# jean-pierreBoth/hnswlib-rs

Measured on AMD Instinct MI355X. Metric: queries/sec (+ recall@10), batched HNSW search, higher is better.
Workload: dtype f32

## Files before the change

### hnswlib-rs_amd/csrc/search_device.hip

```cpp
#include <hip/hip_runtime.h>

#include <algorithm>
#include <chrono>
#include <cmath>
#include <cstdio>
#include <cstdlib>
#include <cstring>
#include <thread>
#include <vector>

#include "hnswio.hpp"
#include "search_device.hpp"
#include "search_kernels.hpp"
#include "worker_pool.hpp"

namespace hnswgpu {

namespace {
Knobs read_knobs() {
    Knobs k;
    auto num = [](const char* name, int unset) { const char* e = std::getenv(name); return e ? std::atoi(e) : unset; };
    auto flag = [](const char* name) { return std::getenv(name) != nullptr; };
    k.hash_bits = num("HNSWGPU_HASH_BITS", -1);
    k.no_sched = flag("HNSWGPU_NO_SCHED");
// ... 614 lines not shown
        HIP_TRY(hipEventElapsedTime(&ms, w.ev_start, w.ev_stop));
        HIP_TRY(hipEventElapsedTime(&ms_main, w.ev_ks, w.ev_stop));
        info.ms = ms;
        info.main_ms = ms_main;
        info.launches = 1;
        publish();
        drain.done = true;
        return OK;
    }

    HIP_TRY(w.tie.ensure(nq * sizeof(uint32_t)));
    HIP_TRY(w.retry[0].ensure(nq * sizeof(uint32_t)));
    HIP_TRY(w.retry[1].ensure(nq * sizeof(uint32_t)));

    int slots = 1;
    while ((uint64_t)slots * 64 < ef) slots *= 2;
    if (slots == 8) slots = 16;
    if (v_.deg_stride > 64u) slots = 16;

    const uint32_t idbits = std::max<uint32_t>(1u, ceil_log2(v_.n));
    const uint64_t expect = ef * std::min<uint64_t>(v_.deg_stride, 64);
    uint32_t tbits = std::min<uint32_t>(14u, std::max<uint32_t>(8u, ceil_log2(expect)));
    {
        std::lock_guard<std::mutex> g(meta_mu_);
        if (adapt_ef_ == ef && adapt_tbits_ != 0) tbits = adapt_tbits_;
    }
    bool env_forced = false;
    const Knobs& kn = knobs();
    if (kn.hash_bits >= 6 && kn.hash_bits <= 14) { tbits = (uint32_t)kn.hash_bits; env_forced = true; }
    const uint32_t tbits_first = tbits;
    const size_t lds_fixed = tile_bytes + IDS_BYTES;
    int table = TABLE_LDS_CELL16;
    bool grown = false;

    const bool scheduled = nq >= 256 && !kn.no_sched;
    if (scheduled) {
        HIP_TRY(w.order.ensure(nq * sizeof(uint32_t)));
        HIP_TRY(kernel_set(kernel_metric()).launch_order(stream, w.pre.as<PreDescent>(), (uint32_t)nq, w.order.as<uint32_t>()));
    }
    uint32_t launches = 0, stop_recorded_after = ~0u;
    uint32_t work = (uint32_t)nq;
    uint32_t n_flagged = 0, n_literal = 0;
    const uint32_t* qlist = scheduled ? w.order.as<uint32_t>() : nullptr;
    int pingpong = 0;
    bool all_done = false;
    const bool pair_auto = (kernel_metric() == DIST_COSINE || kernel_metric() == DIST_DOT) && v_.row_stride <= 32u && strict_ties &&
                           nq >= PAIR_SEARCH_AUTO_MIN_QUERIES;
    if (kn.pair_search > 0 || (kn.pair_search < 0 && pair_auto)) {
        const int tbp = (int)tbits + kn.pair_tbits_delta;
        const uint32_t tb = (uint32_t)std::max(6, std::min<int>(tbp, (int)std::min(14u, idbits + 3u)));
        const bool ok = ef <= 128 && v_.deg_stride <= 64u && kernel_metric() < KM_SIMD8_FIRST && nq >= 512 && idbits >= tb - 3u && idbits - (tb - 3u) <= 13u &&
                        idbits - (tb - 3u) >= 1u;
        if (ok) {
            const KernelSet& ks = kernel_set(kernel_metric());
            SearchArgs a{};
            a.tbits = tb;
            a.restbits = idbits - (tb - 3u);
            a.idbits = idbits;
            a.tile_bytes = tile_bytes;
            a.nrm2 = static_cast<const double*>(d_nrm2_);
            const size_t lds = pair_lds_bytes(tile_bytes, tb, (uint32_t)ef);
            int per_cu = 0;
            HIP_TRY(ks.pair_occupancy(lds, &per_cu));
            if (per_cu >= 1) {
                if (kn.pair_wg_per_cu > 0) per_cu = std::min(per_cu, kn.pair_wg_per_cu);
                const uint64_t npairs = (nq + 1) / 2;
                const uint32_t grid = (uint32_t)std::min<uint64_t>((uint64_t)per_cu * (uint64_t)num_cu_, npairs);
                if (kn.trace_launch)
                    std::fprintf(stderr, "[hnswgpu launch] pair pass: %u queries, %d workgroups per CU, %zu bytes of LDS each, tables 2^%u cells\n",
                                 work, per_cu, lds, tb);
                a.queries = w.qpad.as<float>();
                a.qlist = qlist;
                a.nq = work;
                a.k = (uint32_t)k;
                a.ef = (uint32_t)ef;
                a.work_counter = static_cast<uint32_t*>(w.d_ctrl);
                a.overflow_count = static_cast<uint32_t*>(w.d_ctrl) + 1;
                a.retry_out = w.retry[pingpong].as<uint32_t>();
                a.out_ids = d_out_ids;
                a.out_dists = d_out_dists;
                a.out_layer = d_out_layer;
                a.out_rank = d_out_rank;
                a.out_counts = d_out_counts;
                a.id_stride = layout.id_stride;
                a.dist_stride = layout.dist_stride;
                a.count_stride = layout.count_stride;
                a.stats = stats;
                a.pre = w.pre.as<PreDescent>();
                a.tie_list = w.tie.as<uint32_t>();
                a.pair_ties_to_retry = strict_ties ? 1u : 0u;
                {
                    a.bitmap_words = (v_.n + 31) / 32;
                    const uint64_t slice = (uint64_t)a.bitmap_words * sizeof(uint32_t);
                    const uint64_t blocks = std::min<uint64_t>(2ull * grid, std::max<uint64_t>(2, (4ull << 30) / slice));
                    HIP_TRY(w.bitmap.ensure(blocks * slice));
                    a.bitmap = w.bitmap.as<uint32_t>();
                    a.bitmap_blocks = (uint32_t)blocks;
                }
                HIP_TRY(ks.launch_pair(grid, lds, stream, v_, a, LaunchEvents{w.ev_ks, w.ev_ke}));
                ++launches;
                volatile uint32_t* ctrl = static_cast<volatile uint32_t*>(w.h_ctrl);
                HIP_TRY(hipMemcpyAsync(w.h_ctrl, w.d_ctrl, 24, hipMemcpyDeviceToHost, stream));
                HIP_TRY(hipEventRecord(w.ev_stop, stream));
                stop_recorded_after = launches;
                HIP_TRY(wait_stream(stream));
                n_flagged = ctrl[4];
                info.pair_retries = ctrl[1];
                if (table != TABLE_GLOBAL_BITMAP && !env_forced) {
                    uint32_t next = tbits_first;
                    if ((uint64_t)ctrl[2] * 8 > nq && tbits_first < 14u) next = tbits_first + 1;
                    else if ((uint64_t)ctrl[3] * 32 < nq && tbits_first > 8u) next = tbits_first - 1;
                    std::lock_guard<std::mutex> g(meta_mu_);
                    adapt_ef_ = ef;
                    adapt_tbits_ = next;
                }
                if (ctrl[1] == 0) {
                    all_done = true;
                } else {
                    work = ctrl[1];
                    qlist = w.retry[pingpong].as<uint32_t>();
                    pingpong ^= 1;
                }
            }
        }
    }
    while (!all_done) {
        SearchArgs a{};
        size_t lds = lds_fixed;
        if (table != TABLE_GLOBAL_BITMAP) {
            uint32_t tb = std::max(3u, std::min(tbits, idbits + 3u));
            if (idbits - (tb - 3u) <= 13u) {
                table = TABLE_LDS_CELL16;
                a.restbits = idbits - (tb - 3u);
                lds += (size_t)2 << tb;
            } else {
                table = TABLE_LDS_CELL32;
                lds += (size_t)4 << tb;
            }
            a.tbits = tb;
        }
        a.tile_bytes = tile_bytes;
        a.nrm2 = static_cast<const double*>(d_nrm2_);
        a.idbits = idbits;
        const KernelSet& ks = kernel_set(kernel_metric());
        const bool strict_kernel = strict_ties && table != TABLE_GLOBAL_BITMAP && !kn.no_inkernel;
        if (slots <= (strict_kernel ? HNSW_MERGE_SMAX : HNSW_MERGE_LEAN_SMAX)) {
            a.merge_entries = (uint32_t)slots * 64u + 64u;
            lds += (size_t)a.merge_entries * sizeof(hent_t);
        }
        int per_cu = 0;
        int strict_cap = STRICT_WG_PER_CU;
        if (kn.strict_wg_per_cu > 0) strict_cap = kn.strict_wg_per_cu;
        if (strict_kernel) {
            a.cand_lds = 256;
            if (kn.cand_lds >= 0) {
                a.cand_lds = (uint32_t)std::min(4096, kn.cand_lds);
            } else {
                int occ256 = 0, occ512 = 0;
                HIP_TRY(ks.occupancy(slots, table, true, lds + 256 * sizeof(hent_t), &occ256));
                HIP_TRY(ks.occupancy(slots, table, true, lds + 512 * sizeof(hent_t), &occ512));
                if (std::min(occ512, strict_cap) >= std::min(occ256, strict_cap)) a.cand_lds = 512;
            }
            lds += (size_t)a.cand_lds * sizeof(hent_t);
        }
        HIP_TRY(ks.occupancy(slots, table, strict_kernel, lds, &per_cu));
        if (per_cu < 1) per_cu = 1;
        if (strict_kernel) per_cu = std::min(per_cu, strict_cap);
        if (kn.waves_per_cu > 0) per_cu = std::max(1, std::min(per_cu, kn.waves_per_cu));
        uint32_t grid = (uint32_t)std::min<uint64_t>((uint64_t)per_cu * (uint64_t)num_cu_, work);
        if (kn.trace_launch)
            std::fprintf(stderr, "[hnswgpu launch] %u queries, %d workgroups per CU (strict cap %d), %zu bytes of LDS each (literal heap: %u entries), table 2^%u cells, strict %d, work list %s, slots %d, visited set %s\n",
                         work, per_cu, strict_cap, lds, a.cand_lds, a.tbits, (int)strict_kernel,
                         qlist ? "sorted" : "input order", slots,
                         table == TABLE_LDS_CELL16 ? "cell16" : table == TABLE_LDS_CELL32 ? "cell32" : "bitmap");
        a.queries = w.qpad.as<float>();
        a.qlist = qlist;
        a.nq = work;
        a.k = (uint32_t)k;
        a.ef = (uint32_t)ef;
        a.work_counter = static_cast<uint32_t*>(w.d_ctrl);
        a.overflow_count = static_cast<uint32_t*>(w.d_ctrl) + 1;
        a.retry_out = w.retry[pingpong].as<uint32_t>();
        a.out_ids = d_out_ids;
        a.out_dists = d_out_dists;
        a.out_layer = d_out_layer;
        a.out_rank = d_out_rank;
        a.out_counts = d_out_counts;
        a.id_stride = layout.id_stride;
        a.dist_stride = layout.dist_stride;
        a.count_stride = layout.count_stride;
        a.stats = stats;
        a.pre = w.pre.as<PreDescent>();
        {
            a.bitmap_words = (v_.n + 31) / 32;
            const uint64_t slice = (uint64_t)a.bitmap_words * sizeof(uint32_t);
            uint64_t blocks = std::min<uint64_t>(grid, std::max<uint64_t>(1, (4ull << 30) / slice));
            if (table == TABLE_GLOBAL_BITMAP) grid = (uint32_t)blocks;
            HIP_TRY(w.bitmap.ensure(blocks * slice));
            a.bitmap = w.bitmap.as<uint32_t>();
            a.bitmap_blocks = (uint32_t)blocks;
        }
        a.tie_list = w.tie.as<uint32_t>();
        if (strict_kernel) {
            const uint32_t cap = 4096;
            const uint64_t need = (uint64_t)grid * cap * sizeof(hent_t);
            HIP_TRY(w.cand.ensure(need));
            HIP_TRY(w.oplog.ensure(need));
            a.cand_scratch = w.cand.as<hent_t>();
            a.cand_cap = cap;
            a.oplog = w.oplog.as<hent_t>();
            a.oplog_cap = cap;
            if (kn.exact_first >= 0) a.exact_first = kn.exact_first != 0 ? 1u : 0u;
        }
        if (launches != 0) HIP_TRY(hipMemsetAsync(w.d_ctrl, 0, 16, stream));
        HIP_TRY(ks.launch_search(slots, table, strict_kernel, grid, lds, stream, v_, a,
                                 launches == 0 ? LaunchEvents{w.ev_ks, w.ev_ke} : LaunchEvents{}));
        ++launches;
        volatile uint32_t* ctrl = static_cast<volatile uint32_t*>(w.h_ctrl);
        HIP_TRY(hipMemcpyAsync(w.h_ctrl, w.d_ctrl, 24, hipMemcpyDeviceToHost, stream));
        HIP_TRY(hipEventRecord(w.ev_stop, stream));
        stop_recorded_after = launches;
        HIP_TRY(wait_stream(stream));
        n_flagged = ctrl[4];
        n_literal += ctrl[5];
        if (launches == 1 && table != TABLE_GLOBAL_BITMAP && !env_forced && nq >= 256) {
            uint32_t next = tbits_first;
            if ((uint64_t)ctrl[2] * 8 > nq && tbits_first < 14u) next = tbits_first + 1;
            else if ((uint64_t)ctrl[3] * 32 < nq && tbits_first > 8u) next = tbits_first - 1;
            std::lock_guard<std::mutex> g(meta_mu_);
            adapt_ef_ = ef;
            adapt_tbits_ = next;
        }
        if (ctrl[1] == 0) break;
        work = ctrl[1];
        qlist = w.retry[pingpong].as<uint32_t>();
        pingpong ^= 1;
        if (table == TABLE_GLOBAL_BITMAP) { err = "internal error: bitmap visited set reported an overflow"; return ERR_DEVICE; }
        if (!grown && tbits < 14u) {
            tbits = std::min<uint32_t>(14u, tbits + 2u);
            grown = true;
        } else {
            table = TABLE_GLOBAL_BITMAP;
        }
    }
    info.ties = n_flagged + n_literal;
    if (strict_ties && n_flagged > 0) {
        int rc = run_exact(w, w.qpad.as<float>(), w.tie.as<uint32_t>(), n_flagged, k, ef, nullptr, d_out_ids, d_out_dists, d_out_layer,
                           d_out_rank, d_out_counts, stats, stream, nullptr, err, layout);
        if (rc != OK) return rc;
        ++launches;
    }
    if (stop_recorded_after != launches) {
        HIP_TRY(hipEventRecord(w.ev_stop, stream));
        HIP_TRY(wait_event(w.ev_stop));
    }
    float ms = 0.f, ms_main = 0.f;
    HIP_TRY(hipEventElapsedTime(&ms, w.ev_start, w.ev_stop));
    HIP_TRY(hipEventElapsedTime(&ms_main, w.ev_ks, w.ev_ke));
    info.ms = ms;
    info.main_ms = ms_main;
    info.launches = launches;
    publish();
    drain.done = true;
    return OK;
}

namespace {
struct HostCall {
    const float* queries;
    const float* const* rows;
    float* hq;
    uint64_t d, nq, chunk_rows, task_rows, tasks_per_chunk, n_chunks;
    std::atomic<uint64_t> next_gather{0};
    std::vector<std::atomic<uint32_t>> chunk_left;
    std::atomic<int> phase{0};
    std::atomic<uint64_t> next_unpack{0};
    uint64_t unpack_rows = 256;
    DeviceIndex::HostAnswers answers{};
    const uint32_t* stats = nullptr;
    uint8_t* flags = nullptr;
    const DeviceIndex::AnswerSink* sink = nullptr;
    double us_gather = 0., us_unpack = 0.;

    HostCall(uint64_t n_chunks_) : chunk_left(n_chunks_) {}
    bool gather_one() {
        const uint64_t t = next_gather.fetch_add(1, std::memory_order_relaxed);
        if (t >= n_chunks * tasks_per_chunk) return false;
        const uint64_t c = t / tasks_per_chunk, lo = c * chunk_rows + (t % tasks_per_chunk) * task_rows;
        const uint64_t hi = std::min({nq, (c + 1) * chunk_rows, lo + task_rows});
        const uint64_t row_bytes = d * sizeof(float);
        if (lo < hi) {
            if (queries) std::memcpy(hq + lo * d, queries + lo * d, (hi - lo) * row_bytes);
            else for (uint64_t i = lo; i < hi; ++i) std::memcpy(hq + i * d, rows[i], row_bytes);
        }
        chunk_left[c].fetch_sub(1, std::memory_order_release);
        return true;
    }
    void unpack_all() {
        for (;;) {
            const uint64_t lo = next_unpack.fetch_add(unpack_rows, std::memory_order_relaxed);
            if (lo >= nq) break;
            const uint64_t hi = std::min(nq, lo + unpack_rows);
            if (flags) for (uint64_t i = lo; i < hi; ++i) flags[i] = stats[i * 8 + 3] == 6u ? 1 : 0;
            sink->rows(sink->ctx, answers, lo, hi);
        }
    }
    static std::atomic<int>& calls_in_flight() {
        static std::atomic<int> n{0};
        return n;
    }
    struct InFlight {
        InFlight() { calls_in_flight().fetch_add(1, std::memory_order_relaxed); }
        ~InFlight() { calls_in_flight().fetch_sub(1, std::memory_order_relaxed); }
    };
    struct Spin {
        std::chrono::steady_clock::time_point t0 = std::chrono::steady_clock::now();
        unsigned n = 0;
        bool napping = false;
    };
    static void relax(Spin& w) {
        if (!w.napping) {
#if defined(__x86_64__) || defined(__i386__)
            __builtin_ia32_pause();
#else
            std::this_thread::yield();
// ... 451 lines not shown
```

### hnswlib-rs_amd/csrc/search_kernels.hpp

```cpp
#pragma once
#include <hip/hip_runtime.h>
#include <hip/hip_ext.h>
#include <cstdint>
#include "search_device.hpp"

namespace hnswgpu {

constexpr uint32_t EXPANDED = 0x80000000u;
constexpr uint32_t EMPTY_SLOT = 0xFFFFFFFFu;
constexpr int TABLE_LDS_CELL16 = 0;
constexpr int TABLE_LDS_CELL32 = 1;
constexpr int TABLE_GLOBAL_BITMAP = 2;

constexpr int KM_SIMD8_FIRST = 7;
constexpr int KM_L2_SIMD8 = 7, KM_COSINE_SIMD8 = 8, KM_DOT_SIMD8 = 9, KM_L1_SIMD8 = 10;
constexpr int KM_COUNT = 11;
inline int simd8_kernel_metric(int dist) {
    return dist == DIST_L2 ? KM_L2_SIMD8 : dist == DIST_COSINE ? KM_COSINE_SIMD8 : dist == DIST_DOT ? KM_DOT_SIMD8 : dist == DIST_L1 ? KM_L1_SIMD8 : -1;
}

constexpr uint32_t IDS_BYTES = 64 * 4;

typedef unsigned long long hent_t;

struct PreDescent {
    uint32_t pivot;
    uint32_t dcur_bits;
    uint32_t n_dist;
    uint32_t n_expand;
};
struct DescendArgs {
    const float* src;
    float* qpad;
    PreDescent* pre;
    uint32_t nq;
    uint32_t tile_bytes;
    const double* nrm2;
    uint32_t* ctrl;
    uint32_t ctrl_words;
    uint32_t pair;
};

struct SearchArgs {
    const float* queries;
    const uint32_t* qlist;
    uint32_t nq;
    uint32_t k;
    uint32_t ef;
    uint32_t tbits;
    uint32_t tile_bytes;
    uint32_t idbits;
    uint32_t restbits;
    uint32_t* work_counter;
    uint32_t* overflow_count;
    uint32_t* retry_out;
    uint32_t* bitmap;
    uint32_t bitmap_words;
    uint32_t bitmap_blocks;
    uint32_t* tie_list;
    hent_t* cand_scratch;
    uint32_t cand_cap;
    uint32_t cand_lds;
    uint32_t merge_entries;
    uint32_t exact_first;
    uint32_t pair_ties_to_retry;
    hent_t* oplog;
    uint32_t oplog_cap;
    const double* nrm2;
    uint64_t* out_ids;
    float* out_dists;
    uint8_t* out_layer;
    int32_t* out_rank;
    uint32_t* out_counts;
    const PreDescent* pre;
    uint32_t* stats;
    uint32_t id_stride, dist_stride, count_stride;
};

struct ExactArgs {
    hent_t* heaps;
    uint64_t heap_stride;
    uint32_t cand_cap;
    uint32_t r_lds_cap;
    uint32_t cand_lds;
    const uint32_t* allow;
};

struct BuildLists {
    uint32_t* lists[NB_LAYER_MAX];
    uint32_t stride[NB_LAYER_MAX];
};
struct BuildArgs {
    const float* vec;
    uint32_t row_stride;
    const uint32_t* lists[NB_LAYER_MAX];
    uint32_t stride[NB_LAYER_MAX];
    const uint8_t* level;
    const uint32_t* slot0;
    uint32_t first, count;
    uint32_t entry, entry_level;
    uint32_t layer_mask;
    uint32_t ef_c;
    uint32_t tbits, idbits, restbits, tile_bytes;
    uint32_t* bitmap;
    uint32_t bitmap_words, bitmap_blocks;
    uint32_t* work_counter;
    uint32_t* fail_count;
    uint32_t* out_ids;
    float* out_d;
    uint32_t* out_n;
    uint32_t* hit_ids;
    float* hit_d;
    const double* nrm2;
};

struct SelectArgs {
    const float* vec;
    uint32_t row_stride;
    uint32_t tile_bytes;
    const double* nrm2;
    uint32_t* cand_ids;
    const float* cand_d;
    const uint32_t* cand_n;
    uint32_t ef_c;
    const uint16_t* slot_nb;
    uint32_t n_slots;
    uint32_t sel_stride;
    uint32_t keep_pruned;
    uint32_t* sel_ids;
    float* sel_d;
    uint32_t* sel_n;
    uint32_t* work_counter;
};

constexpr uint32_t LAB_PUSH = 1, LAB_POP = 2, LAB_PUSH_LANES = 3, LAB_INSERT = 4, LAB_MERGE = 5, LAB_BATCH = 6, LAB_VISIT = 7;
struct LaneLabArgs {
    const uint32_t* ops;
    uint32_t n_ops;
    const uint32_t* lanes;
    uint32_t mode;
    uint32_t p0, p1, p2;
    hent_t* scratch;
    uint32_t scratch_cap;
    uint32_t* out;
    uint32_t out_cap;
};
hipError_t launch_lane_lab(hipStream_t stream, size_t lds, const LaneLabArgs& a);

struct LaunchEvents {
    hipEvent_t start = nullptr;
    hipEvent_t stop = nullptr;
};

struct KernelSet {
    hipError_t (*launch_search)(int slots, int table, bool strict, uint32_t grid, size_t lds, hipStream_t stream,
                                const DeviceIndexView& ix, const SearchArgs& a, LaunchEvents ev);
    hipError_t (*occupancy)(int slots, int table, bool strict, size_t lds, int* per_cu);
    hipError_t (*launch_pair)(uint32_t grid, size_t lds, hipStream_t stream, const DeviceIndexView& ix, const SearchArgs& a, LaunchEvents ev);
    hipError_t (*pair_occupancy)(size_t lds, int* per_cu);
    hipError_t (*launch_exact)(int ns, uint32_t grid, size_t lds, hipStream_t stream, const DeviceIndexView& ix,
                               const SearchArgs& a, const ExactArgs& x);
    hipError_t (*exact_occupancy)(int ns, size_t lds, int* per_cu);
    hipError_t (*launch_descend)(uint32_t grid, hipStream_t stream, const DeviceIndexView& ix, const DescendArgs& a, LaunchEvents ev);
    hipError_t (*descend_occupancy)(size_t lds, bool pair, int* per_cu);
    hipError_t (*launch_order)(hipStream_t stream, const PreDescent* pre, uint32_t n, uint32_t* order);
    hipError_t (*launch_eval_matrix)(hipStream_t stream, const float* queries, uint32_t nq, const float* rows, uint32_t n_rows,
                                     const double* nrm2, float* out, uint32_t row_stride, uint32_t d, uint32_t nf, bool pairs);
    hipError_t (*launch_build_search)(int slots, uint32_t grid, size_t lds, hipStream_t stream, const BuildArgs& a);
    hipError_t (*build_occupancy)(int slots, size_t lds, int* per_cu);
    hipError_t (*launch_build_select)(uint32_t grid, size_t lds, hipStream_t stream, const SelectArgs& a);
};
#ifndef HNSW_MERGE_SMAX
#define HNSW_MERGE_SMAX 4
#endif
#ifndef HNSW_MERGE_LEAN_SMAX
#define HNSW_MERGE_LEAN_SMAX 2
// ... 26 lines not shown
```

### hnswlib-rs_amd/csrc/search_kernels.inc

```
#pragma clang fp contract(off)
#include <type_traits>
#include "ln_f32.hpp"

#ifndef HNSW_LB_WAVES
#define HNSW_LB_WAVES 5
#endif
#ifndef HNSW_MERGE_LISTS
#define HNSW_MERGE_LISTS 1
#endif
#ifndef HNSW_LB_WAVES_STRICT
#define HNSW_LB_WAVES_STRICT 4
#endif
#ifndef HNSW_LB_DESCEND
#define HNSW_LB_DESCEND 6
#endif
#ifndef HNSW_DPP_ASM
#define HNSW_DPP_ASM 1
#endif
#ifndef HNSW_PIPE_ROWS
#define HNSW_PIPE_ROWS 1
#endif
#ifndef HNSW_DEEP_G2
#define HNSW_DEEP_G2 1
#endif
// ... 1304 lines not shown
template <int S>
struct SortedR {
    hent_t s[S];
    uint32_t len;
};
template <int S>
__device__ HNSW_COLD SortedR<S> literal_return_points(const void* kargs, uint32_t log_len) {
    const kernargs_t ka = uniform_kernargs(kargs);
    const int lane = (int)threadIdx.x;
    log_len = (uint32_t)__builtin_amdgcn_readfirstlane((int)log_len);
    const uint32_t ef = ka->a.ef;
    const hent_t* oplog = ka->a.oplog + (size_t)blockIdx.x * ka->a.oplog_cap;
    hfence();
    RegHeap<S> RR;
#pragma unroll
    for (int s = 0; s < S; ++s) RR.s[s] = 0ull;
    uint32_t lenR = 0;
    for (uint32_t base = 0; base < log_len; base += 64) {
        const uint32_t li = base + (uint32_t)lane;
        const hent_t mine = li < log_len ? __hip_atomic_load(oplog + li, __ATOMIC_RELAXED, __HIP_MEMORY_SCOPE_AGENT) : 0ull;
        const uint32_t cntb = log_len - base < 64u ? log_len - base : 64u;
        for (uint32_t t = 0; t < cntb; ++t) {
            const hent_t e = readlane_h(mine, (int)t);
            if (e == LOG_EXPAND) continue;
            if (lenR == RegHeap<S>::CAP) {
                RR.push_then_pop_full(e, lane);
            } else {
                RR.push(lenR, e, lane);
                if (lenR > ef) (void)RR.pop(lenR, lane);
            }
        }
    }
    uint32_t end = lenR;
    while (end > 1u) {
        end -= 1;
        const hent_t r0 = RR.get(0u), re = RR.get(end);
        RR.set(0u, re, lane);
        RR.set(end, r0, lane);
        RR.sift_down_range(end, lane);
    }
    SortedR<S> out;
#pragma unroll
    for (int s = 0; s < S; ++s) out.s[s] = RR.s[s];
    out.len = lenR < ef ? lenR : ef;
    return out;
}


template <int S>
struct QueryEnd {
    float rd[S];
    uint32_t ri[S];
    uint32_t q, len, status, out_status, n_dist, n_expand, n_ids, t_start, flags;
    uint32_t feedback;
#if HNSW_PHASE_TIMING
    uint32_t ph[4], ph_miss;
#endif
};
__device__ __forceinline__ void put_id(uint64_t* base, uint32_t stride, size_t o, uint64_t v) {
    *reinterpret_cast<uint64_t*>(reinterpret_cast<unsigned char*>(base) + o * stride) = v;
}
__device__ __forceinline__ void put_dist(float* base, uint32_t stride, size_t o, float v) {
    *reinterpret_cast<float*>(reinterpret_cast<unsigned char*>(base) + o * stride) = v;
}
__device__ __forceinline__ void put_answer(uint64_t* ids, uint32_t id_stride, float* dists, uint32_t dist_stride, size_t o, uint64_t id, float d) {
    if (id_stride == 16u && dist_stride == 16u && reinterpret_cast<unsigned char*>(dists) == reinterpret_cast<unsigned char*>(ids) + 8) {
        *reinterpret_cast<uint4*>(reinterpret_cast<unsigned char*>(ids) + o * 16u) = make_uint4((uint32_t)id, (uint32_t)(id >> 32), __float_as_uint(d), 0u);
    } else {
        put_id(ids, id_stride, o, id);
        put_dist(dists, dist_stride, o, d);
    }
}
__device__ __forceinline__ void put_count(uint32_t* base, uint32_t stride, size_t q, uint32_t v) {
    *reinterpret_cast<uint32_t*>(reinterpret_cast<unsigned char*>(base) + q * stride) = v;
}
template <int S>
__device__ __attribute__((noinline)) void finish_query(const void* kargs, QueryEnd<S> e) {
    const kernargs_t ka = uniform_kernargs(kargs);
    const int lane = (int)threadIdx.x;
    const uint32_t q = (uint32_t)__builtin_amdgcn_readfirstlane((int)e.q), len = (uint32_t)__builtin_amdgcn_readfirstlane((int)e.len);
    uint32_t status = (uint32_t)__builtin_amdgcn_readfirstlane((int)e.status);
    uint32_t out_status = (uint32_t)__builtin_amdgcn_readfirstlane((int)e.out_status);
    const uint32_t feedback = (uint32_t)__builtin_amdgcn_readfirstlane((int)e.feedback);
    const uint32_t k = ka->a.k;
    uint32_t* const counters = ka->a.overflow_count;
    if (out_status == 3u && lane == 0) atomicAdd(counters + 4, 1u);
    if (status == 2u) {
        uint32_t* const tie_list = ka->a.tie_list;
        if (tie_list != nullptr && lane == 0) tie_list[atomicAdd(counters + 3, 1u)] = q;
    }
    if (status != 0u) out_status = status;
    if (status != 1u) {
        const uint32_t cnt = len < k ? len : k;
        uint64_t* const out_ids = ka->a.out_ids;
        float* const out_dists = ka->a.out_dists;
        uint8_t* const out_layer = ka->a.out_layer;
        int32_t* const out_rank = ka->a.out_rank;
        const uint64_t* const origin_id = ka->ix.origin_id;
        const uint32_t id_stride = ka->a.id_stride, dist_stride = ka->a.dist_stride;
#pragma unroll
        for (int s = 0; s < S; ++s) {
            const uint32_t j = (uint32_t)s * 64u + (uint32_t)lane;
            if (j < k) {
                const size_t o = (size_t)q * k + j;
                if (j < cnt) {
                    const uint32_t flat = e.ri[s] & ~EXPANDED;
                    uint32_t l = 0;
                    while (l + 1 < NB_LAYER_MAX && flat >= ka->ix.layer_offset[l + 1]) ++l;
                    put_answer(out_ids, id_stride, out_dists, dist_stride, o, origin_id[flat], e.rd[s]);
                    if (out_layer) out_layer[o] = (uint8_t)l;
                    if (out_rank) out_rank[o] = (int32_t)(flat - ka->ix.layer_offset[l]);
                } else {
                    put_answer(out_ids, id_stride, out_dists, dist_stride, o, 0ull, 0.f);
                    if (out_layer) out_layer[o] = 0;
                    if (out_rank) out_rank[o] = 0;
                }
            }
        }
        if (lane == 0) put_count(ka->a.out_counts, ka->a.count_stride, q, cnt);
    } else if (lane == 0) {
        const uint32_t slot = atomicAdd(counters, 1u);
        ka->a.retry_out[slot] = q;
    }
    if (lane == 0 && (feedback & 4u) != 0u) {
        if (feedback & 1u) atomicAdd(counters + 1, 1u);
        if (feedback & 2u) atomicAdd(counters + 2, 1u);
    }
    if (lane == 0) {
        uint32_t* st = ka->a.stats + (size_t)q * 8;
        st[0] = e.n_dist; st[1] = e.n_expand; st[2] = e.n_ids; st[3] = out_status;
        st[4] = e.t_start; st[5] = (uint32_t)wall_clock64(); st[6] = (e.flags & 4u) ? 1u : 0u;
        st[7] = (e.flags & 3u) | ((ka->a.pre[q].n_expand & 0xFFu) << 8) | (ka->a.pre[q].n_dist << 16);
#if HNSW_PHASE_TIMING
#if HNSW_PHASE_TIMING == 2
        st[7] = e.ph[0]; st[2] = e.ph[1]; st[6] = e.ph[3]; st[0] = 0u;
#else
        st[7] = e.ph[0]; st[3] = e.ph[1]; st[2] = e.ph[2]; st[6] = e.ph[3];
        st[0] = e.ph_miss;
#endif
#endif
    }
}


struct DescentOut {
    uint32_t pivot;
    float dcur;
    uint32_t n_dist, n_expand, n_ids;
};
__device__ __attribute__((noinline, unused)) DescentOut load_descent(const void* kargs, uint32_t q) {
    const kernargs_t ka = uniform_kernargs(kargs);
    q = (uint32_t)__builtin_amdgcn_readfirstlane((int)q);
    const PreDescent pd = ka->a.pre[q];
    DescentOut o{pd.pivot, __uint_as_float(pd.dcur_bits), pd.n_dist, pd.n_expand, pd.n_dist - 1u};
    hent_t* oplog = ka->a.oplog;
    const uint32_t cap = ka->a.oplog_cap;
    if (oplog != nullptr && cap != 0u && threadIdx.x == 0)
        __hip_atomic_store(oplog + (size_t)blockIdx.x * cap, hmake(o.dcur, o.pivot), __ATOMIC_RELAXED, __HIP_MEMORY_SCOPE_AGENT);
    return o;
}


template <int METRIC, int TABLE>
__device__ __attribute__((noinline)) uint32_t begin_query(const void* kargs, bool first) {
    extern __shared__ __attribute__((aligned(16))) unsigned char lds_raw[];
    const kernargs_t ka = uniform_kernargs(kargs);
    const int lane = (int)threadIdx.x;
    uint32_t wi = 0;
    if (__builtin_amdgcn_readfirstlane((int)first) != 0) {
        wi = blockIdx.x;
    } else {
        if (lane == 0) wi = atomicAdd(ka->a.work_counter, 1u);
        wi = readlane_u(wi, 0) + gridDim.x;
    }
    if (wi >= ka->a.nq) return EMPTY_SLOT;
    const uint32_t* qlist = ka->a.qlist;
    const uint32_t q = qlist ? qlist[wi] : wi;
    const uint32_t row_stride = ka->ix.row_stride;
    stage_query<METRIC>(reinterpret_cast<float4*>(lds_raw), ka->a.queries + (size_t)q * row_stride, row_stride, lane, ka->ix.d);
    if constexpr (TABLE == TABLE_GLOBAL_BITMAP) {
        const uint32_t words = ka->a.bitmap_words;
        uint32_t* bitmap = ka->a.bitmap + (size_t)blockIdx.x * words;
        for (uint32_t i = (uint32_t)lane; i < words; i += 64) bitmap[i] = 0u;
    } else {
        uint32_t* table = reinterpret_cast<uint32_t*>(lds_raw + ka->a.tile_bytes + IDS_BYTES);
        const uint32_t cells = 1u << ka->a.tbits;
        const uint32_t words = TABLE == TABLE_LDS_CELL16 ? cells >> 1 : cells;
        const uint32_t fill = TABLE == TABLE_LDS_CELL16 ? 0u : EMPTY_SLOT;
        for (uint32_t i = (uint32_t)lane; i < words; i += 64) table[i] = fill;
    }
    __syncthreads();
    return q;
}
template <int TABLE>
__device__ __attribute__((noinline)) void migrate_table_to_bitmap(const void* kargs) {
    extern __shared__ __attribute__((aligned(16))) unsigned char lds_raw[];
    const kernargs_t ka = uniform_kernargs(kargs);
    const int lane = (int)threadIdx.x;
    const uint32_t words = ka->a.bitmap_words, restbits = ka->a.restbits, idbits = ka->a.idbits;
    uint32_t* bitmap = ka->a.bitmap + (size_t)blockIdx.x * words;
    const uint32_t* table = reinterpret_cast<const uint32_t*>(lds_raw + ka->a.tile_bytes + IDS_BYTES);
    const uint32_t table_cells = 1u << ka->a.tbits;
    for (uint32_t i = (uint32_t)lane; i < words; i += 64) bitmap[i] = 0u;
    __syncthreads();
    for (uint32_t i = (uint32_t)lane; i < table_cells; i += 64) {
        uint32_t id = EMPTY_SLOT;
        if constexpr (TABLE == TABLE_LDS_CELL16) {
            const uint32_t half = (table[i >> 1] >> ((i & 1u) * 16u)) & 0xFFFFu;
            if (half != 0u) {
                const uint32_t bdisp = (half & 0x7FFFu) >> restbits;
                const uint32_t rest = half & ((1u << restbits) - 1u);
                const uint32_t home = ((i >> 3) - bdisp) & ((table_cells >> 3) - 1u);
                id = unmix_id((home << restbits) | rest, idbits);
            }
        } else if constexpr (TABLE == TABLE_LDS_CELL32) {
            id = table[i];
        }
        if (id != EMPTY_SLOT) atomicOr(&bitmap[id >> 5], 1u << (id & 31u));
    }
    __syncthreads();
}

template <int S>
__device__ __forceinline__ bool final_order_ambiguous(const float (&rd)[S], uint32_t len, uint32_t k, float taint_w, int lane) {
    const uint32_t kk = k < len ? k : len;
    if (kk == 0u) return false;
    unsigned long long bad = 0ull;
#pragma unroll
    for (int s = 0; s < S; ++s) {
        const uint32_t j = (uint32_t)s * 64u + (uint32_t)lane;
        const float nxt = __shfl_down(rd[s], 1);
        const float edge = s + 1 < S ? r_dist_at<S>(rd, (uint32_t)(s + 1) * 64u) : INFINITY;
        const float nd = lane == 63 ? edge : nxt;
        bad |= __ballot(j < kk && j + 1u < len && rd[s] == nd);
    }
    return bad != 0ull || r_dist_at<S>(rd, kk - 1u) == taint_w;
}

template <int METRIC, int S, int TABLE, bool STRICT>
__global__ __launch_bounds__(64, STRICT ? (S >= 16 ? 2 : S == 4 && HNSW_PIPE_ROWS != 0 ? 3 : HNSW_LB_WAVES_STRICT) : (S >= 16 ? 4 : HNSW_LB_WAVES)) void hnsw_search_kernel(DeviceIndexView ix, SearchArgs a) {
    extern __shared__ __attribute__((aligned(16))) unsigned char lds_raw[];
    const void* const kargs = (const void*)__builtin_amdgcn_kernarg_segment_ptr();
    float4* tile = reinterpret_cast<float4*>(lds_raw);
    uint32_t* ids_lds = reinterpret_cast<uint32_t*>(lds_raw + a.tile_bytes);
    uint32_t* table = reinterpret_cast<uint32_t*>(lds_raw + a.tile_bytes + IDS_BYTES);
    const int lane = (int)threadIdx.x;
    const uint32_t table_cells = 1u << a.tbits;
    const uint32_t table_words = TABLE == TABLE_LDS_CELL16 ? table_cells >> 1 : table_cells;
    const uint32_t table_limit = table_cells - (table_cells >> 2);
    uint32_t* bitmap = blockIdx.x < a.bitmap_blocks ? a.bitmap + (size_t)blockIdx.x * a.bitmap_words : nullptr;
    constexpr bool ONE_BATCH = S < 16;
    const bool single_batch = ONE_BATCH || ix.deg_stride <= 64u;
    const uint32_t nbatch = ONE_BATCH ? 1u : (ix.deg_stride + 63u) >> 6;
    const nrm_ptr_t nrm2 = (nrm_ptr_t)a.nrm2;
    bool use_bm = TABLE == TABLE_GLOBAL_BITMAP;
    const bool strict = STRICT && a.cand_scratch != nullptr && a.oplog != nullptr && TABLE != TABLE_GLOBAL_BITMAP;

    auto visit = [&](uint32_t id) __attribute__((always_inline)) -> int {
        if (TABLE == TABLE_GLOBAL_BITMAP || use_bm) return visit_bitmap(bitmap, id);
        if constexpr (TABLE == TABLE_LDS_CELL16) return visit_cell16(table, a.tbits, a.idbits, a.restbits, id);
        else return visit_cell32(table, a.tbits, id);
    };
    auto migrate_to_bitmap = [&]() __attribute__((always_inline)) {
        migrate_table_to_bitmap<TABLE>(kargs);
        use_bm = true;
    };

    bool first_item = true;
    for (;;) {
        const uint32_t q = (uint32_t)__builtin_amdgcn_readfirstlane((int)begin_query<METRIC, TABLE>(kargs, first_item));
        first_item = false;
        if (q == EMPTY_SLOT) break;
        const uint32_t t_start = (uint32_t)wall_clock64();

        uint32_t n_dist = 1, n_expand = 0, n_ids = 0, status = 0, n_visited = 1;
        bool flag_tie = false;
#if HNSW_PHASE_TIMING
        uint32_t ph[4] = {0, 0, 0, 0};
        uint32_t ph_miss = 0;
#endif
        use_bm = TABLE == TABLE_GLOBAL_BITMAP;

        const DescentOut dsc = load_descent(kargs, q);
        const uint32_t pivot = (uint32_t)__builtin_amdgcn_readfirstlane((int)dsc.pivot);
        const float dcur = __int_as_float(__builtin_amdgcn_readfirstlane(__float_as_int(dsc.dcur)));
        n_dist += (uint32_t)__builtin_amdgcn_readfirstlane((int)dsc.n_dist);
        n_expand += (uint32_t)__builtin_amdgcn_readfirstlane((int)dsc.n_expand);
        n_ids += (uint32_t)__builtin_amdgcn_readfirstlane((int)dsc.n_ids);

        float de = INFINITY;
        uint32_t idc = 0u;
        auto gather_batch = [&](uint32_t id, unsigned long long any_id) __attribute__((always_inline)) -> uint32_t {
            const bool valid = id != EMPTY_SLOT;
            n_ids += popc64(any_id);
            if (TABLE != TABLE_GLOBAL_BITMAP && !use_bm && n_visited + 64 > table_limit) {
                if (bitmap == nullptr) { status = 1; return 0u; }
                migrate_to_bitmap();
            }
            bool fresh = false, to_insert = false;
            Probe16 pr{};
            if (TABLE == TABLE_LDS_CELL16 && !use_bm) {
                int t = 1;
                if (valid) t = cell16_test(table, a.restbits, a.idbits, id, pr);
                if (__ballot(t == 2) != 0ull) {
                    int vr = 0;
                    if (t == 2) vr = visit_cell16(table, a.tbits, a.idbits, a.restbits, id);
                    if (__ballot(vr == 2) != 0ull) {
                        if (bitmap == nullptr) { status = 1; return 0u; }
                        migrate_to_bitmap();
                        if (vr == 2) vr = visit_bitmap(bitmap, id);
                        if (t == 0) { t = 2; vr = visit_bitmap(bitmap, id); }
                    }
                    if (t == 2) fresh = vr == 1;
                }
                if (t == 0) { fresh = true; to_insert = true; }
            } else {
                int vr = 0;
                if (valid) vr = visit(id);
                if (__ballot(vr == 2) != 0ull) {
                    if (use_bm || bitmap == nullptr) { status = 1; return 0u; }
                    migrate_to_bitmap();
                    if (vr == 2) vr = visit_bitmap(bitmap, id);
                }
                fresh = vr == 1;
            }
            const unsigned long long fm = __ballot(fresh);
            const uint32_t nf = popc64(fm);
            if (nf == 0u) return 0u;
            n_visited += nf;
            n_dist += nf;
            wave_lds_fence();
            if (fresh) ids_lds[popc64(fm & lanemask_lt(lane))] = id;
            wave_lds_fence();
            idc = (uint32_t)lane < nf ? ids_lds[lane] : 0u;
            PH_T(gt1);
            int irc = 1;
            de = batch_dist<METRIC, HNSW_DEEP_G2 != 0 && STRICT && S <= 2, HNSW_PIPE_ROWS != 0 && STRICT && S == 4>(ix.vec, ix.row_stride, ix.d, nrm2, tile, ids_lds, nf, lane, [&]() __attribute__((always_inline)) {
                if constexpr (TABLE == TABLE_LDS_CELL16) {
                    if (to_insert) irc = cell16_insert(table, a.tbits, a.restbits, pr);
                }
            });
            PH_T(gt2);
#if HNSW_PHASE_TIMING == 1
            PH_ACC(1, gt1, gt2);
#endif
            if constexpr (TABLE == TABLE_LDS_CELL16) {
                if (__ballot(irc == 2) != 0ull) {
                    if (bitmap == nullptr) { status = 1; return 0u; }
                    migrate_to_bitmap();
                    if (irc == 2) (void)visit_bitmap(bitmap, id);
                }
            }
            return nf;
        };

        hent_t* oplog = nullptr;
        bool log_ok = false;
        uint32_t log_len = 0;
        if constexpr (STRICT) {
            if (strict) { oplog = a.oplog + (size_t)blockIdx.x * a.oplog_cap; log_ok = true; log_len = 1; }
        }
        auto log_put = [&](hent_t e) __attribute__((always_inline)) {
            if constexpr (STRICT) {
                if (log_ok) {
                    if (log_len < a.oplog_cap) {
                        if (lane == 0) __hip_atomic_store(oplog + log_len, e, __ATOMIC_RELAXED, __HIP_MEMORY_SCOPE_AGENT);
                        log_len += 1;
                    } else {
                        log_ok = false;
                    }
                }
            }
        };
        bool pend_marker = false;
        unsigned long long pend_mask = 0ull;
        auto log_flush = [&]() __attribute__((always_inline)) {
            if constexpr (STRICT) {
                if (pend_marker || pend_mask != 0ull) {
                    if (log_ok) {
                        const uint32_t n_acc = popc64(pend_mask);
                        const uint32_t need = n_acc + (pend_marker ? 1u : 0u);
                        if (log_len + need <= a.oplog_cap) {
                            if (pend_marker && lane == 0) __hip_atomic_store(oplog + log_len, LOG_EXPAND, __ATOMIC_RELAXED, __HIP_MEMORY_SCOPE_AGENT);
                            const uint32_t at = log_len + (pend_marker ? 1u : 0u) +
                                                __builtin_amdgcn_mbcnt_hi((uint32_t)(pend_mask >> 32), __builtin_amdgcn_mbcnt_lo((uint32_t)pend_mask, 0u));
                            if (((pend_mask >> lane) & 1ull) != 0ull)
                                __hip_atomic_store(oplog + at, hmake(de, idc), __ATOMIC_RELAXED, __HIP_MEMORY_SCOPE_AGENT);
                            log_len += need;
                        } else {
                            log_ok = false;
                        }
                    }
                    pend_marker = false;
                    pend_mask = 0ull;
                }
            }
        };

        float rd[S];
        uint32_t ri[S];
#pragma unroll
        for (int s = 0; s < S; ++s) { rd[s] = 0.f; ri[s] = 0u; }
        uint32_t len = 1;
        bool tie_any = false;
        uint32_t ghost = 0;
        float ghost_w = 0.f;
        float taint_w = -1.f;
        uint32_t spec_for = EMPTY_SLOT, spec_ids = EMPTY_SLOT;
        hent_t* merge_buf = reinterpret_cast<hent_t*>(table + (TABLE == TABLE_GLOBAL_BITMAP ? 0u : table_words));
        auto merge_list = [&](unsigned long long cand) __attribute__((always_inline)) -> bool {
#include "merge_list_body.inc"
            if (tie_here) tie_any = true;
            ghost = 0u;
            pend_mask |= acc;
            return true;
        };
        if (lane == 0) { rd[0] = dcur; ri[0] = pivot; }
        if (lane == 0) (void)visit(pivot);
        uint32_t lenC = 0, log_replayed = 0;
        bool literal_used = false;
        uint32_t out_status = 0;
        for (;;) {
            PH_T(pt0);
            const int cj = r_next<S>(ri, len, lane);
            bool amb = false;
            if (tie_any) {
                if (cj >= 0) {
                    const float dcj = r_dist_at<S>(rd, (uint32_t)cj);
                    uint32_t n_equal = 0;
#pragma unroll
                    for (int s = 0; s < S; ++s) {
                        const uint32_t j = (uint32_t)s * 64u + (uint32_t)lane;
                        n_equal += popc64(__ballot(j < len && rd[s] == dcj && (ri[s] & EXPANDED) == 0u));
                    }
                    amb = n_equal >= 2u || (ghost > 0u && dcj == ghost_w);
                } else {
                    amb = ghost > 0u;
                }
            }
            if constexpr (STRICT) {
                if (strict && a.exact_first != 0u) amb = true;
            }
            uint32_t c = 0;
            bool popped = false;
            if (__builtin_expect(amb, 0)) {
                if (STRICT && strict && log_ok) log_flush();
                if (STRICT && strict && log_ok) {
#if HNSW_PHASE_TIMING == 2
                    const unsigned long long lt0 = clock64();
#endif
                    const LiteralPop lp = literal_candidate_pop<TABLE>(kargs, log_replayed, log_len, lenC);
#if HNSW_PHASE_TIMING == 2
                    ph[1] += (uint32_t)(clock64() - lt0);
                    ph[3] += (uint32_t)__builtin_amdgcn_readfirstlane((int)lp.n_ops);
                    ph[0] += (uint32_t)__builtin_amdgcn_readfirstlane((int)lp.t_pops);
#endif
                    lenC = (uint32_t)__builtin_amdgcn_readfirstlane((int)lp.lenC);
                    log_replayed = log_len;
                    const hent_t ce = readlane_h(lp.ce, 0);
                    const int prc = __builtin_amdgcn_readfirstlane(lp.rc);
                    if (prc == 0) {
                        literal_used = true;
                        popped = true;
                        log_put(LOG_EXPAND);
                        if (log_ok) log_replayed = log_len;
                        if (-hkey(ce) > r_worst<S>(rd, len)) break;
                        c = hid(ce);
                        unsigned long long found = 0ull;
#pragma unroll
                        for (int s = 0; s < S; ++s) {
                            const uint32_t j = (uint32_t)s * 64u + (uint32_t)lane;
                            const bool hit = j < len && ri[s] == c;
                            if (hit) ri[s] |= EXPANDED;
                            found |= __ballot(hit);
                        }
                        if (found == 0ull && ghost > 0u) ghost -= 1u;
                    } else if (prc == 1) {
                        break;
                    } else {
                        log_ok = false;
                        flag_tie = true;
                    }
                } else {
                    flag_tie = true;
                }
            }
            if (!popped) {
                if (cj < 0) break;
                c = r_id_at<S>(ri, cj);
#pragma unroll
                for (int s = 0; s < S; ++s)
                    if ((cj >> 6) == s && lane == (cj & 63)) ri[s] |= EXPANDED;
            }
            n_expand += 1;
            const uint32_t* nrow = ix.nbr0 + (size_t)c * ix.deg_stride;
            for (uint32_t bi = 0; bi < nbatch; ++bi) {
                const uint32_t j = bi * 64u + (uint32_t)lane;
                uint32_t id;
                if (single_batch && spec_for == c) id = spec_ids;
                else id = j < ix.deg_stride ? nrow[j] : EMPTY_SLOT;
#if HNSW_PHASE_TIMING == 1
                if (!(single_batch && spec_for == c)) ph_miss += 1;
#endif
                const unsigned long long any_id = __ballot(id != EMPTY_SLOT);
                log_flush();
                if (bi == 0u && !popped) pend_marker = true;
                if (single_batch) {
                    const int nj = r_next<S>(ri, len, lane);
                    if (nj >= 0) {
                        spec_for = r_id_at<S>(ri, nj);
                        spec_ids = (uint32_t)lane < ix.deg_stride ? ix.nbr0[(size_t)spec_for * ix.deg_stride + (uint32_t)lane] : EMPTY_SLOT;
                    } else {
                        spec_for = EMPTY_SLOT;
                    }
                }
                PH_T(pt1);
#if HNSW_PHASE_TIMING == 1
                PH_ACC(0, pt0, pt1);
#endif
                if (any_id == 0ull) break;
                const uint32_t nf = gather_batch(id, any_id);
                PH_T(pt3);
                PH_ACC(2, pt1, pt3);
                if (status != 0) break;
                if (nf == 0u) continue;
                float worst = r_worst<S>(rd, len);
                unsigned long long cand = nf >= 64u ? ~0ull : (1ull << nf) - 1ull;
                if (len >= a.ef) cand &= __ballot(de < worst);
                if constexpr ((S == 1 || (S <= HNSW_MERGE_SMAX && (STRICT || S <= HNSW_MERGE_LEAN_SMAX))) && HNSW_MERGE_LISTS != 0) {
                    if (len == a.ef && popc64(cand) >= (uint32_t)HNSW_MERGE_LISTS && merge_list(cand)) cand = 0ull;
                }
                while (cand != 0ull) {
                    const int jl = ctz64(cand);
                    const float xd = readlane_f(de, jl);
                    if (xd < worst || len < a.ef) {
                        const uint32_t xi = readlane_u(idc, jl);
                        pend_mask |= 1ull << jl;
                        const bool was_full = len == a.ef;
                        uint32_t last_if = 0u;
                        if (was_full) last_if = r_id_flag_at<S>(ri, a.ef - 1u);
                        if (r_insert<S>(rd, ri, len, a.ef, xd, xi, lane)) tie_any = true;
                        const float nw = r_worst<S>(rd, len);
                        if (was_full) {
                            if (nw == worst) {
                                taint_w = nw;
                                if ((last_if & EXPANDED) == 0u) { ghost += 1u; ghost_w = nw; }
                            } else {
                                ghost = 0u;
                            }
                        }
                        worst = nw;
                    }
                    cand &= cand - 1ull;
                }
                PH_T(pt4);
#if HNSW_PHASE_TIMING == 1
                PH_ACC(3, pt3, pt4);
#endif
            }
            if (status != 0) break;
        }
        log_flush();
        if (literal_used) out_status = 3;

        if constexpr (STRICT) {
            if (__builtin_expect(strict && status == 0 && !flag_tie && tie_any && final_order_ambiguous<S>(rd, len, a.k, taint_w, lane), 0)) {
                if (!log_ok) {
                    flag_tie = true;
                } else {
                    const SortedR<S> sr = literal_return_points<S>(kargs, log_len);
                    len = (uint32_t)__builtin_amdgcn_readfirstlane((int)sr.len);
#pragma unroll
                    for (int s = 0; s < S; ++s) {
                        rd[s] = hkey(sr.s[s]);
                        ri[s] = hid(sr.s[s]);
                    }
                    out_status = 3;
                }
            }
        } else {
            if (status == 0 && tie_any && !flag_tie && final_order_ambiguous<S>(rd, len, a.k, taint_w, lane)) flag_tie = true;
        }
        if (status == 0 && flag_tie) status = 2;
        {
            QueryEnd<S> e;
#pragma unroll
            for (int s = 0; s < S; ++s) { e.rd[s] = rd[s]; e.ri[s] = ri[s]; }
            e.q = q; e.len = len; e.status = status; e.out_status = out_status;
            e.n_dist = n_dist; e.n_expand = n_expand; e.n_ids = n_ids; e.t_start = t_start;
            e.flags = (tie_any ? 1u : 0u) | (literal_used ? 2u : 0u) | (use_bm ? 4u : 0u);
            e.feedback = (use_bm ? 1u : 0u) | (n_visited > (table_limit >> 1) ? 2u : 0u) | (TABLE != TABLE_GLOBAL_BITMAP ? 4u : 0u);
#if HNSW_PHASE_TIMING
            e.ph[0] = ph[0]; e.ph[1] = ph[1]; e.ph[2] = ph[2]; e.ph[3] = ph[3]; e.ph_miss = ph_miss;
#endif
            finish_query<S>(kargs, e);
        }
        __syncthreads();
    }
}


template <int METRIC, int NS>
__global__ __launch_bounds__(64, 4) void hnsw_search_exact_kernel(DeviceIndexView ix, SearchArgs a, ExactArgs x) {
    RegHeap<(NS > 0 ? NS : 1)> RR;
    extern __shared__ __attribute__((aligned(16))) unsigned char lds_raw[];
    float4* tile = reinterpret_cast<float4*>(lds_raw);
    uint32_t* ids_lds = reinterpret_cast<uint32_t*>(lds_raw + a.tile_bytes);
    const int lane = (int)threadIdx.x;
    uint32_t* bitmap = a.bitmap + (size_t)blockIdx.x * a.bitmap_words;
    const nrm_ptr_t nrm2 = (nrm_ptr_t)a.nrm2;
    hent_t* lds_heaps = reinterpret_cast<hent_t*>(lds_raw + a.tile_bytes + IDS_BYTES);
    hent_t* glb = x.heaps + (size_t)blockIdx.x * x.heap_stride;
    const uint32_t r_lds = a.ef + 2u <= x.r_lds_cap ? a.ef + 2u : x.r_lds_cap;
    const HeapMem R{lds_heaps, glb, r_lds};
    const HeapMem Cq{lds_heaps + r_lds, glb + (a.ef + 2u), x.cand_lds};
    const bool filtered = x.allow != nullptr;
    auto allowed = [&](uint32_t flat) __attribute__((always_inline)) -> bool { return (x.allow[flat >> 5] >> (flat & 31u)) & 1u; };
    auto r_push_capped = [&](uint32_t& len, hent_t item) __attribute__((always_inline)) {
        if constexpr (NS > 0) {
            if (len == RegHeap<(NS > 0 ? NS : 1)>::CAP) { RR.push_then_pop_full(item, lane); return; }
            RR.push(len, item, lane);
            if (len > a.ef) (void)RR.pop(len, lane);
        } else {
            heap_push(R, len, item, lane);
            if (len > a.ef) (void)heap_pop(R, len, lane);
        }
    };
    auto r_any_refused = [&](uint32_t len) __attribute__((always_inline)) -> bool {
        unsigned long long m = 0ull;
        if constexpr (NS > 0) {
#pragma unroll
            for (int k = 0; k < (NS > 0 ? NS : 1); ++k) {
                const uint32_t i = 64u * (uint32_t)k + (uint32_t)lane;
                m |= __ballot(i < len && !allowed(hid(RR.s[k])));
            }
        } else {
            for (uint32_t i0 = 0; i0 < len; i0 += 64) {
                const uint32_t i = i0 + (uint32_t)lane;
                m |= __ballot(i < len && !allowed(hid(hload(R, i < len ? i : 0u))));
            }
        }
        return m != 0ull;
    };
    auto r_get = [&](uint32_t i) __attribute__((always_inline)) -> hent_t {
        if constexpr (NS > 0) return RR.get(i);
        else return hload(R, i);
    };

    for (;;) {
        uint32_t wi = 0;
        if (lane == 0) wi = atomicAdd(a.work_counter, 1u);
        wi = readlane_u(wi, 0);
        if (wi >= a.nq) break;
        const uint32_t q = a.qlist ? a.qlist[wi] : wi;
        const uint32_t t_start = (uint32_t)wall_clock64();
        stage_query<METRIC>(tile, a.queries + (size_t)q * ix.row_stride, ix.row_stride, lane, ix.d);
        for (uint32_t i = (uint32_t)lane; i < a.bitmap_words; i += 64) bitmap[i] = 0u;
        __syncthreads();
        uint32_t n_dist = 1, n_expand = 0, n_ids = 0, status = 0;

        const PreDescent pd = a.pre[q];
        const uint32_t pivot = pd.pivot;
        const float dcur = __uint_as_float(pd.dcur_bits);
        n_dist += pd.n_dist; n_expand += pd.n_expand; n_ids += pd.n_dist - 1u;

        uint32_t lenR = 0, lenC = 0;
        bool returned = false;
        if (lane == 0) (void)visit_bitmap(bitmap, pivot);
        __syncthreads();
        heap_push(Cq, lenC, hmake(-dcur, pivot), lane);
        r_push_capped(lenR, hmake(dcur, pivot));
        const bool single_batch = ix.deg_stride <= 64u;
        uint32_t spec_for = EMPTY_SLOT, spec_ids = EMPTY_SLOT;
        while (lenC > 0u && status == 0 && !returned) {
            const hent_t c = lenC < 32768u ? heap_pop3(Cq, lenC, lane) : heap_pop(Cq, lenC, lane);
            if (lenR == 0u) { status = 6; break; }
            float worst = hkey(r_get(0u));
            if (-hkey(c) > worst) {
                if (!filtered) break;
                if (lenR >= a.ef) {
                    if (r_any_refused(lenR)) {
                        if (lenR == 1u) lenR = 0u;
                        else { status = 7; break; }
                    }
                }
            }
            n_expand += 1;
            const uint32_t* nrow = ix.nbr0 + (size_t)hid(c) * ix.deg_stride;
            const uint32_t nbatch = (ix.deg_stride + 63u) >> 6;
            for (uint32_t bi = 0; bi < nbatch; ++bi) {
                const uint32_t j = bi * 64u + (uint32_t)lane;
                uint32_t id;
                if (single_batch && spec_for == hid(c)) id = spec_ids;
                else id = j < ix.deg_stride ? nrow[j] : EMPTY_SLOT;
                const bool valid = id != EMPTY_SLOT;
                const unsigned long long vm = __ballot(valid);
                if (single_batch) {
                    if (lenC > 0u) {
                        spec_for = hid(hload(Cq, 0u));
                        spec_ids = (uint32_t)lane < ix.deg_stride ? ix.nbr0[(size_t)spec_for * ix.deg_stride + (uint32_t)lane] : EMPTY_SLOT;
                    } else {
                        spec_for = EMPTY_SLOT;
                    }
                }
                if (vm == 0ull) break;
                n_ids += popc64(vm);
                const bool fresh = valid && visit_bitmap(bitmap, id) == 1;
                const unsigned long long fm = __ballot(fresh);
                const uint32_t nf = popc64(fm);
                if (nf == 0u) continue;
                if (lenR == 0u) { returned = true; break; }
                n_dist += nf;
                wave_lds_fence();
                if (fresh) ids_lds[popc64(fm & lanemask_lt(lane))] = id;
                wave_lds_fence();
                const uint32_t idc = (uint32_t)lane < nf ? ids_lds[lane] : 0u;
                bool alw = true;
                if (filtered) alw = (uint32_t)lane < nf && allowed(idc);
                const float de = batch_dist<METRIC>(ix.vec, ix.row_stride, ix.d, nrm2, tile, ids_lds, nf, lane);
                const unsigned long long allow_m = __ballot(alw && (uint32_t)lane < nf);
                unsigned long long acc = 0ull;
                unsigned long long rest = nf >= 64u ? ~0ull : ((1ull << nf) - 1ull);
// ... 422 lines not shown
```

Baseline: 9.386 million.

## Stage strict-mode op log in LDS and flush to global in 64-entry blocks

Op-log entries in the strict kernel are now first written to a ring buffer in LDS and copied to global memory one whole 64-entry block at a time, with a sync of the partial block before any literal replay reads the log. This replaces scattered per-entry relaxed atomic stores to global memory with coalesced block stores. The literal-heap size heuristic also gains a 384-entry option so the extra LDS for the stage does not cost occupancy. The added LDS and fences may lower workgroups per CU, and the change only affects the strict path.

```diff
diff --git a/hnswlib-rs_amd/csrc/search_device.hip b/hnswlib-rs_amd/csrc/search_device.hip
--- a/hnswlib-rs_amd/csrc/search_device.hip
+++ b/hnswlib-rs_amd/csrc/search_device.hip
@@ -790,14 +790,18 @@
         int strict_cap = STRICT_WG_PER_CU;
         if (kn.strict_wg_per_cu > 0) strict_cap = kn.strict_wg_per_cu;
         if (strict_kernel) {
+            lds += (size_t)LOG_STAGE * sizeof(hent_t);
             a.cand_lds = 256;
             if (kn.cand_lds >= 0) {
                 a.cand_lds = (uint32_t)std::min(4096, kn.cand_lds);
             } else {
-                int occ256 = 0, occ512 = 0;
+                int occ256 = 0;
                 HIP_TRY(ks.occupancy(slots, table, true, lds + 256 * sizeof(hent_t), &occ256));
-                HIP_TRY(ks.occupancy(slots, table, true, lds + 512 * sizeof(hent_t), &occ512));
-                if (std::min(occ512, strict_cap) >= std::min(occ256, strict_cap)) a.cand_lds = 512;
+                for (uint32_t top : {512u, 384u}) {
+                    int occ = 0;
+                    HIP_TRY(ks.occupancy(slots, table, true, lds + top * sizeof(hent_t), &occ));
+                    if (std::min(occ, strict_cap) >= std::min(occ256, strict_cap)) { a.cand_lds = top; break; }
+                }
             }
             lds += (size_t)a.cand_lds * sizeof(hent_t);
         }
@@ -807,8 +811,8 @@
         if (kn.waves_per_cu > 0) per_cu = std::max(1, std::min(per_cu, kn.waves_per_cu));
         uint32_t grid = (uint32_t)std::min<uint64_t>((uint64_t)per_cu * (uint64_t)num_cu_, work);
         if (kn.trace_launch)
-            std::fprintf(stderr, "[hnswgpu launch] %u queries, %d workgroups per CU (strict cap %d), %zu bytes of LDS each (literal heap: %u entries), table 2^%u cells, strict %d, work list %s, slots %d, visited set %s\n",
-                         work, per_cu, strict_cap, lds, a.cand_lds, a.tbits, (int)strict_kernel,
+            std::fprintf(stderr, "[hnswgpu launch] %u queries, %d workgroups per CU (strict cap %d), %zu bytes of LDS each (literal heap: %u entries, log stage: %u), table 2^%u cells, strict %d, work list %s, slots %d, visited set %s\n",
+                         work, per_cu, strict_cap, lds, a.cand_lds, strict_kernel ? LOG_STAGE : 0u, a.tbits, (int)strict_kernel,
                          qlist ? "sorted" : "input order", slots,
                          table == TABLE_LDS_CELL16 ? "cell16" : table == TABLE_LDS_CELL32 ? "cell32" : "bitmap");
         a.queries = w.qpad.as<float>();
diff --git a/hnswlib-rs_amd/csrc/search_kernels.hpp b/hnswlib-rs_amd/csrc/search_kernels.hpp
--- a/hnswlib-rs_amd/csrc/search_kernels.hpp
+++ b/hnswlib-rs_amd/csrc/search_kernels.hpp
@@ -22,6 +22,12 @@
 constexpr uint32_t IDS_BYTES = 64 * 4;
 
 typedef unsigned long long hent_t;
+
+#ifndef HNSW_LOG_STAGE
+#define HNSW_LOG_STAGE 128
+#endif
+constexpr uint32_t LOG_STAGE = HNSW_LOG_STAGE;
+static_assert(LOG_STAGE >= 64 && LOG_STAGE % 64 == 0, "the log stage holds whole blocks of 64 entries");
 
 struct PreDescent {
     uint32_t pivot;
diff --git a/hnswlib-rs_amd/csrc/search_kernels.inc b/hnswlib-rs_amd/csrc/search_kernels.inc
--- a/hnswlib-rs_amd/csrc/search_kernels.inc
+++ b/hnswlib-rs_amd/csrc/search_kernels.inc
@@ -1480,12 +1480,7 @@
     const kernargs_t ka = uniform_kernargs(kargs);
     q = (uint32_t)__builtin_amdgcn_readfirstlane((int)q);
     const PreDescent pd = ka->a.pre[q];
-    DescentOut o{pd.pivot, __uint_as_float(pd.dcur_bits), pd.n_dist, pd.n_expand, pd.n_dist - 1u};
-    hent_t* oplog = ka->a.oplog;
-    const uint32_t cap = ka->a.oplog_cap;
-    if (oplog != nullptr && cap != 0u && threadIdx.x == 0)
-        __hip_atomic_store(oplog + (size_t)blockIdx.x * cap, hmake(o.dcur, o.pivot), __ATOMIC_RELAXED, __HIP_MEMORY_SCOPE_AGENT);
-    return o;
+    return DescentOut{pd.pivot, __uint_as_float(pd.dcur_bits), pd.n_dist, pd.n_expand, pd.n_dist - 1u};
 }
 
 
@@ -1683,42 +1678,64 @@
         };
 
         hent_t* oplog = nullptr;
+        hent_t* log_stage = nullptr;
         bool log_ok = false;
         uint32_t log_len = 0;
         if constexpr (STRICT) {
-            if (strict) { oplog = a.oplog + (size_t)blockIdx.x * a.oplog_cap; log_ok = true; log_len = 1; }
-        }
+            if (strict) {
+                oplog = a.oplog + (size_t)blockIdx.x * a.oplog_cap;
+                log_stage = reinterpret_cast<hent_t*>(table + table_words) + a.merge_entries + a.cand_lds;
+                log_ok = true;
+                log_len = 1;
+                if (lane == 0) log_stage[0] = hmake(dcur, pivot);
+            }
+        }
+        auto log_store_block = [&](uint32_t base, uint32_t n) __attribute__((always_inline)) {
+            wave_lds_fence();
+            if ((uint32_t)lane < n)
+                __hip_atomic_store(oplog + base + (uint32_t)lane, log_stage[(base + (uint32_t)lane) % LOG_STAGE], __ATOMIC_RELAXED, __HIP_MEMORY_SCOPE_AGENT);
+        };
+        auto log_append = [&](bool marker, unsigned long long mask, hent_t mine) __attribute__((always_inline)) {
+            const uint32_t need = popc64(mask) + (marker ? 1u : 0u);
+            if (log_len + need > a.oplog_cap) {
+                log_ok = false;
+                return;
+            }
+            const uint32_t old = log_len;
+            const uint32_t at = old + (marker ? 1u : 0u) +
+                                __builtin_amdgcn_mbcnt_hi((uint32_t)(mask >> 32), __builtin_amdgcn_mbcnt_lo((uint32_t)mask, 0u));
+            const bool has = ((mask >> lane) & 1ull) != 0ull;
+            if (marker && lane == 0) log_stage[old % LOG_STAGE] = LOG_EXPAND;
+            log_len = old + need;
+            if constexpr (LOG_STAGE >= 128) {
+                if (has) log_stage[at % LOG_STAGE] = mine;
+                for (uint32_t b = old >> 6; b < (log_len >> 6); ++b) log_store_block(b << 6, 64u);
+            } else {
+                const uint32_t edge = (old | 63u) + 1u;
+                if (has && at < edge) log_stage[at % LOG_STAGE] = mine;
+                if (log_len >= edge) {
+                    log_store_block(edge - 64u, 64u);
+                    wave_lds_fence();
+                    if (has && at >= edge) log_stage[at % LOG_STAGE] = mine;
+                    if (log_len >= edge + 64u) log_store_block(edge, 64u);
+                }
+            }
+        };
         auto log_put = [&](hent_t e) __attribute__((always_inline)) {
+            (void)e;
             if constexpr (STRICT) {
-                if (log_ok) {
-                    if (log_len < a.oplog_cap) {
-                        if (lane == 0) __hip_atomic_store(oplog + log_len, e, __ATOMIC_RELAXED, __HIP_MEMORY_SCOPE_AGENT);
-                        log_len += 1;
-                    } else {
-                        log_ok = false;
-                    }
-                }
-            }
+                if (log_ok) log_append(true, 0ull, 0ull);
+            }
+        };
+        auto log_sync = [&]() __attribute__((always_inline)) {
+            if constexpr (STRICT) log_store_block(log_len & ~63u, log_len & 63u);
         };
         bool pend_marker = false;
         unsigned long long pend_mask = 0ull;
         auto log_flush = [&]() __attribute__((always_inline)) {
             if constexpr (STRICT) {
                 if (pend_marker || pend_mask != 0ull) {
-                    if (log_ok) {
-                        const uint32_t n_acc = popc64(pend_mask);
-                        const uint32_t need = n_acc + (pend_marker ? 1u : 0u);
-                        if (log_len + need <= a.oplog_cap) {
-                            if (pend_marker && lane == 0) __hip_atomic_store(oplog + log_len, LOG_EXPAND, __ATOMIC_RELAXED, __HIP_MEMORY_SCOPE_AGENT);
-                            const uint32_t at = log_len + (pend_marker ? 1u : 0u) +
-                                                __builtin_amdgcn_mbcnt_hi((uint32_t)(pend_mask >> 32), __builtin_amdgcn_mbcnt_lo((uint32_t)pend_mask, 0u));
-                            if (((pend_mask >> lane) & 1ull) != 0ull)
-                                __hip_atomic_store(oplog + at, hmake(de, idc), __ATOMIC_RELAXED, __HIP_MEMORY_SCOPE_AGENT);
-                            log_len += need;
-                        } else {
-                            log_ok = false;
-                        }
-                    }
+                    if (log_ok) log_append(pend_marker, pend_mask, hmake(de, idc));
                     pend_marker = false;
                     pend_mask = 0ull;
                 }
@@ -1774,6 +1791,7 @@
             if (__builtin_expect(amb, 0)) {
                 if (STRICT && strict && log_ok) log_flush();
                 if (STRICT && strict && log_ok) {
+                    log_sync();
 #if HNSW_PHASE_TIMING == 2
                     const unsigned long long lt0 = clock64();
 #endif
@@ -1896,6 +1914,7 @@
                 if (!log_ok) {
                     flag_tie = true;
                 } else {
+                    log_sync();
                     const SortedR<S> sr = literal_return_points<S>(kargs, log_len);
                     len = (uint32_t)__builtin_amdgcn_readfirstlane((int)sr.len);
 #pragma unroll
```

Measured after the change: 6.611 million. -29.6%, worse.
